# BogdanDIA/gr-dvbt

Hardware: AMD Instinct MI355X
Metric: RX Msamples/s (baseband in -> TS out) (higher is better)
Workload: dtype u8 (Viterbi/RS) + f32 (front end)

## Files before the change

gr_dvbt_amd/csrc/k_symbol8k.hpp:

```cpp
#pragma once
#include "k_frontend.hpp"
#include "k_backend.hpp"

namespace dvbt {

#ifndef S8_EXP
#define S8_EXP 0
#endif
#ifndef S8_MIN_WAVES
#define S8_MIN_WAVES 4
#endif
constexpr int S8_N = 8192, S8_T = 512, S8_PAY = 6048, S8_NCP = 177, S8_NTPS = 68, S8_ZL = 688;
constexpr int S8_IT = (S8_PAY + S8_T - 1) / S8_T;
#ifndef S8_TOP_N
#define S8_TOP_N 6
#endif
constexpr int S8_TOP = S8_TOP_N;
constexpr size_t S8_SMALL_BYTES = DEMOD_NP * 8 + 2 * 128 * 8 + 64 * 8 + 192 * 4 + 16 * 4 + 64 * 4 + 192 * 2 + 64 + 16;
constexpr size_t S8_LDS_BYTES = (size_t)((S8_EXP & 128) ? S8_N / 2 : S8_N) * 8 + S8_SMALL_BYTES;
#ifndef S8_WG_PER_CU
#define S8_WG_PER_CU 2
#endif
inline int s8_grid(int cus) { return S8_WG_PER_CU * cus; }

__device__ __forceinline__ int s8_swz1(int a) { return a ^ ((a >> 5) & 15) ^ (((a >> 9) & 1) << 4); }
__device__ __forceinline__ int s8_swz2(int b) { return b ^ ((b >> 4) & 15); }

__device__ __forceinline__ void s8_fill_ptab(float2 *pt, const SymMeta &m, int t)
{
  const double thA = (double)m.ph_base + m.incA, thB = (double)m.ph_base + (double)m.sw * (m.incA - m.incB) + m.incB;
  double ang;
  if (t < 16) ang = 512.0 * t * m.incA;
  else if (t < 32) ang = 512.0 * (t - 16) * m.incB;
  else if (t < 48) ang = thA + 32.0 * (t - 32) * m.incA;
  else if (t < 64) ang = thB + 32.0 * (t - 48) * m.incB;
  else if (t < 96) ang = (double)(t - 64) * m.incA;
  else ang = (double)(t - 96) * m.incB;
  float sn, cs; sincosf(wrap_pi(ang), &sn, &cs);
  pt[t] = make_float2(cs, sn);
}

typedef float v2f __attribute__((ext_vector_type(2)));
__device__ __forceinline__ v2f s8_v(float2 a) { return (v2f){a.x, a.y}; }
__device__ __forceinline__ float2 s8_f(v2f a) { return make_float2(a.x, a.y); }
__device__ __forceinline__ v2f s8_cmul(v2f a, v2f b)
{
  v2f p, r;
  asm("v_pk_mul_f32 %0, %1, %2 op_sel:[1,1] op_sel_hi:[1,0]" : "=v"(p) : "v"(a), "v"(b));
  asm("v_pk_fma_f32 %0, %1, %2, %3 op_sel:[0,0,0] op_sel_hi:[0,1,1] neg_lo:[0,0,1]" : "=v"(r) : "v"(a), "v"(b), "v"(p));
  return r;
}
__device__ __forceinline__ v2f s8_add_mi(v2f a, v2f b)
{ v2f r; asm("v_pk_add_f32 %0, %1, %2 op_sel:[0,1] op_sel_hi:[1,0] neg_hi:[0,1]" : "=v"(r) : "v"(a), "v"(b)); return r; }
__device__ __forceinline__ v2f s8_add_pi(v2f a, v2f b)
{ v2f r; asm("v_pk_add_f32 %0, %1, %2 op_sel:[0,1] op_sel_hi:[1,0] neg_lo:[0,1]" : "=v"(r) : "v"(a), "v"(b)); return r; }
__device__ __forceinline__ v2f s8_mul_mi(v2f y)
{ v2f r; asm("v_pk_add_f32 %0, %1, 0 op_sel:[1,0] op_sel_hi:[0,1] neg_hi:[1,0]" : "=v"(r) : "v"(y)); return r; }
#define S8_MULK(name, m1, m2) \
  __device__ __forceinline__ v2f name(v2f y, v2f K) { v2f p, r; \
    asm("v_pk_mul_f32 %0, %1, %2 " m1 : "=v"(p) : "v"(y), "v"(K)); \
    asm("v_pk_fma_f32 %0, %1, %2, %3 " m2 : "=v"(r) : "v"(y), "v"(K), "v"(p)); return r; }
S8_MULK(s8_mul_c_ms, "op_sel:[0,0] op_sel_hi:[1,0]", "op_sel:[1,1,0] op_sel_hi:[0,1,1] neg_hi:[1,0,0]")
S8_MULK(s8_mul_s_mc, "op_sel:[0,1] op_sel_hi:[1,1]", "op_sel:[1,0,0] op_sel_hi:[0,0,1] neg_hi:[1,0,0]")
S8_MULK(s8_mul_mc_s, "op_sel:[0,0] op_sel_hi:[1,0] neg_lo:[0,1] neg_hi:[0,1]", "op_sel:[1,1,0] op_sel_hi:[0,1,1] neg_lo:[1,0,0]")
S8_MULK(s8_mul_ms_mc, "op_sel:[0,1] op_sel_hi:[1,1] neg_lo:[0,1] neg_hi:[0,1]", "op_sel:[1,0,0] op_sel_hi:[0,0,1] neg_hi:[1,0,0]")
S8_MULK(s8_mul_mc_ms, "op_sel:[0,0] op_sel_hi:[1,0] neg_lo:[0,1] neg_hi:[0,1]", "op_sel:[1,1,0] op_sel_hi:[0,1,1] neg_hi:[1,0,0]")
#undef S8_MULK
__device__ __forceinline__ v2f s8_mul_h_mh(v2f y, v2f H)
{
  v2f t, r;
  asm("v_pk_add_f32 %0, %1, %1 op_sel:[0,1] op_sel_hi:[1,0] neg_hi:[0,1]" : "=v"(t) : "v"(y));
  asm("v_pk_mul_f32 %0, %1, %2" : "=v"(r) : "v"(t), "v"(H));
  return r;
}
__device__ __forceinline__ v2f s8_mul_mh_mh(v2f y, v2f H)
{
  v2f t, r;
  asm("v_pk_add_f32 %0, %1, %1 op_sel:[0,1] op_sel_hi:[1,0] neg_lo:[0,1]" : "=v"(t) : "v"(y));
  asm("v_pk_mul_f32 %0, %1, %2 neg_lo:[0,1] neg_hi:[0,1]" : "=v"(r) : "v"(t), "v"(H));
  return r;
}
struct S8Roots { v2f K8, K16, K316, H; };
__device__ __forceinline__ S8Roots s8_roots()
{
  S8Roots R;
  R.K8 = (v2f){0.92387953251128674f, 0.38268343236508977f}; R.K16 = (v2f){0.98078528040323043f, 0.19509032201612825f};
  R.K316 = (v2f){0.83146961230254524f, 0.55557023301960218f}; R.H = (v2f){0.70710678118654752f, 0.70710678118654752f};
  return R;
}
__device__ __forceinline__ void s8_bfly4(v2f a0, v2f a1, v2f a2, v2f a3, v2f &y0, v2f &y1, v2f &y2, v2f &y3)
{
  const v2f s02 = a0 + a2, d02 = a0 - a2, s13 = a1 + a3, d13 = a1 - a3;
  y0 = s02 + s13; y2 = s02 - s13; y1 = s8_add_mi(d02, d13); y3 = s8_add_pi(d02, d13);
}
__device__ __forceinline__ void s8_dft16(v2f (&a)[16], const S8Roots &R)
{
  v2f t[16];
#pragma unroll
  for (int rp = 0; rp < 4; rp++) {
    v2f y0, y1, y2, y3;
    s8_bfly4(a[rp], a[rp + 4], a[rp + 8], a[rp + 12], y0, y1, y2, y3);
    t[rp] = y0;
    if (rp == 0) { t[4] = y1; t[8] = y2; t[12] = y3; }
    else if (rp == 1) { t[5] = s8_mul_c_ms(y1, R.K8); t[9] = s8_mul_h_mh(y2, R.H); t[13] = s8_mul_s_mc(y3, R.K8); }
    else if (rp == 2) { t[6] = s8_mul_h_mh(y1, R.H); t[10] = s8_mul_mi(y2); t[14] = s8_mul_mh_mh(y3, R.H); }
    else { t[7] = s8_mul_s_mc(y1, R.K8); t[11] = s8_mul_mh_mh(y2, R.H); t[15] = s8_mul_mc_s(y3, R.K8); }
  }
#pragma unroll
  for (int k1 = 0; k1 < 4; k1++) {
    v2f y0, y1, y2, y3;
    s8_bfly4(t[k1 * 4], t[k1 * 4 + 1], t[k1 * 4 + 2], t[k1 * 4 + 3], y0, y1, y2, y3);
    a[k1] = y0; a[k1 + 4] = y1; a[k1 + 8] = y2; a[k1 + 12] = y3;
  }
}
__device__ __forceinline__ void s8_twiddle16(v2f (&a)[16], v2f w1)
{
  v2f w[16];
  w[1] = w1;
  w[2] = s8_cmul(w[1], w[1]); w[3] = s8_cmul(w[2], w[1]); w[4] = s8_cmul(w[2], w[2]); w[5] = s8_cmul(w[4], w[1]); w[6] = s8_cmul(w[3], w[3]);
  w[7] = s8_cmul(w[4], w[3]); w[8] = s8_cmul(w[4], w[4]); w[9] = s8_cmul(w[8], w[1]); w[10] = s8_cmul(w[5], w[5]); w[11] = s8_cmul(w[8], w[3]);
  w[12] = s8_cmul(w[6], w[6]); w[13] = s8_cmul(w[8], w[5]); w[14] = s8_cmul(w[7], w[7]); w[15] = s8_cmul(w[8], w[7]);
#pragma unroll
  for (int k = 1; k < 16; k++) a[k] = s8_cmul(a[k], w[k]);
}
template <int B> __device__ __forceinline__ v2f s8_mul_w32(v2f u, const S8Roots &R)
{
  if (B == 1) return s8_mul_c_ms(u, R.K16); if (B == 2) return s8_mul_c_ms(u, R.K8); if (B == 3) return s8_mul_c_ms(u, R.K316);
  if (B == 4) return s8_mul_h_mh(u, R.H);
  if (B == 5) return s8_mul_s_mc(u, R.K316); if (B == 6) return s8_mul_s_mc(u, R.K8); if (B == 7) return s8_mul_s_mc(u, R.K16);
  if (B == 8) return s8_mul_mi(u);
  if (B == 9) return s8_mul_ms_mc(u, R.K16); if (B == 10) return s8_mul_ms_mc(u, R.K8); if (B == 11) return s8_mul_ms_mc(u, R.K316);
  if (B == 12) return s8_mul_mh_mh(u, R.H);
  if (B == 13) return s8_mul_mc_ms(u, R.K316); if (B == 14) return s8_mul_mc_ms(u, R.K8); if (B == 15) return s8_mul_mc_ms(u, R.K16);
  return u;
}

template <int CTRL> __device__ __forceinline__ float s8_dpp(float v) { return __builtin_bit_cast(float, __builtin_amdgcn_update_dpp(0, __builtin_bit_cast(int, v), CTRL, 0xf, 0xf, true)); }
__device__ __forceinline__ float s8_row_sum(float v)
{ v += s8_dpp<0xB1>(v); v += s8_dpp<0x4E>(v); v += s8_dpp<0x141>(v); v += s8_dpp<0x140>(v); return v; }
__device__ __forceinline__ float s8_row_max(float v)
{ v = fmaxf(v, s8_dpp<0xB1>(v)); v = fmaxf(v, s8_dpp<0x4E>(v)); v = fmaxf(v, s8_dpp<0x141>(v)); v = fmaxf(v, s8_dpp<0x140>(v)); return v; }
__device__ __forceinline__ float s8_quad_max(float v) { v = fmaxf(v, s8_dpp<0xB1>(v)); return fmaxf(v, s8_dpp<0x4E>(v)); }

constexpr float S8_MARGIN = 2.0e-5f, S8_REACH = 4.0f;
__device__ __forceinline__ bool s8_demap_cell(v2f e, float inv_step, float half_n, float top, int &idx)
{
  const float gx = __builtin_fmaf(e.x, inv_step, half_n), gy = __builtin_fmaf(e.y, inv_step, half_n);
  const float cx = __builtin_amdgcn_fmed3f(gx, 0.5f, top), cy = __builtin_amdgcn_fmed3f(gy, 0.5f, top);
  const float fx = floorf(cx), fy = floorf(cy);
  const bool ok = fabsf((cx - fx) - 0.5f) < 0.5f - S8_MARGIN && fabsf((cy - fy) - 0.5f) < 0.5f - S8_MARGIN &&
                  fabsf(gx - cx) < S8_REACH && fabsf(gy - cy) < S8_REACH;
  idx = (int)fx * 8 + (int)fy;
  return ok;
}

typedef int s8_i4 __attribute__((ext_vector_type(4)));
__device__ v2f s8_raw_buffer_load_v2f32(s8_i4 rsrc, int voffset, int soffset, int aux) __asm("llvm.amdgcn.raw.buffer.load.v2f32");
__device__ __forceinline__ s8_i4 s8_rsrc(const v2f *base)
{
  const unsigned long long a = (unsigned long long)base;
  s8_i4 r;
  r.x = __builtin_amdgcn_readfirstlane((int)(unsigned)a); r.y = __builtin_amdgcn_readfirstlane((int)(unsigned)(a >> 32)) & 0xffff;
  r.z = 0x7fffffff; r.w = 0x00020000;
  return r;
}
__device__ __forceinline__ s8_i4 s8_rsrc_lim(const v2f *iq, long long low, long long avail)
{
  s8_i4 r = s8_rsrc(iq + low);
  long long bytes = (avail - low) * 8; bytes = bytes < 0 ? 0 : (bytes > 0x7fffffffll ? 0x7fffffffll : bytes);
  r.z = __builtin_amdgcn_readfirstlane((int)bytes);
  return r;
}
__device__ __forceinline__ v2f s8_sample(s8_i4 rsrc, int i, int tid) { return s8_raw_buffer_load_v2f32(rsrc, tid * 8, i * S8_T * 8, 0); }

template <bool TAPS, bool DRIFT> __global__ __launch_bounds__(S8_T, S8_MIN_WAVES) void symbol8k_kernel(const float2 *__restrict__ iq_, FrontParams p, const RxState *st,
                                                           const SymMeta *__restrict__ meta, const float2 *__restrict__ tw, float2 *__restrict__ acq_tap,
                                                           float2 *__restrict__ fft_tap, DemodTables T, float2 *__restrict__ eq_tap,
                                                           float2 *__restrict__ tpsval, SymInfo *__restrict__ info, InnerParams ip,
                                                           const float2 *__restrict__ points, const unsigned char *__restrict__ label_tab,
                                                           uint8_t *__restrict__ labels, int *__restrict__ ticket,
                                                           const float *__restrict__ drift, const int *__restrict__ drift_flags, float *__restrict__ csi_tap)
{
  if ((drift_flags[1] != 0) != DRIFT) return;
  extern __shared__ __attribute__((aligned(16))) unsigned char smem_raw[];
  v2f *x = reinterpret_cast<v2f *>((S8_EXP & 128) ? smem_raw + S8_SMALL_BYTES : smem_raw);
  v2f *gtab = (S8_EXP & 128) ? reinterpret_cast<v2f *>(smem_raw) : x + S8_N;
  float2 *ptab = reinterpret_cast<float2 *>(gtab + DEMOD_NP);
  float2 *pts = ptab + 256;
  float *s_known = reinterpret_cast<float *>(pts + 64);
  float *s_cfo = s_known + 192;
  float *s_pat = s_cfo + 16;
  short *s_cpil = reinterpret_cast<short *>(s_pat + 64);
  unsigned char *label_of = reinterpret_cast<unsigned char *>(s_cpil + 192);
  int *s_tkt = reinterpret_cast<int *>(label_of + 64);
  const v2f *iq = reinterpret_cast<const v2f *>(iq_);
  constexpr int N = S8_N, zl = S8_ZL;
  const int tid0 = threadIdx.x, tid = tid0, cp = p.cp;
  const int nsym = st->n_symbols, call0 = st->call0;
  if (tid == 0) s_tkt[0] = atomicAdd(ticket, 1);
  __syncthreads();
  int s = __builtin_amdgcn_readfirstlane(s_tkt[0]);
  if (s >= nsym) return;

  if (tid < 64) { pts[tid] = points[tid]; label_of[tid] = label_tab[tid]; }
  if (tid < S8_NCP) { s_cpil[tid] = T.cpilot[tid]; if (tid < S8_NCP - 1) s_known[tid] = T.known_diff[tid]; }
  const v2f w1A = s8_v(tw[tid]), w1B = s8_v(tw[16 * (tid & 31)]);
  const int tps_c = tid < S8_NTPS ? T.tps[tid] : 0;
  float pat_ref = 0.f;
  if (tid >= 256) { const int q = tid - 256, j = q & 15, pat = (q >> 4) & 3; if (j < 10) pat_ref = T.pilot_ref[3 * pat + 12 * j]; }
  const float half_n = 0.5f * (float)ip.nlev, top = (float)ip.nlev - 0.5f;

  int cur_mod = 0, s_prev = s;

  SymMeta m = meta[s];
  v2f vin[16];
  {
    const long long low = (long long)(call0 + s) * (N + cp) + m.cp_start - N + 1;
    const s8_i4 rs = s8_rsrc_lim(iq, low, p.avail);
#pragma unroll
    for (int i = S8_TOP; i < 16; i++) vin[i] = s8_sample(rs, i, tid);
  }
  if (tid < 128) s8_fill_ptab(ptab, m, tid);
  int par = 0;
  __syncthreads();

  for (;;) {
    int tid = tid0;
    asm volatile("" : "+v"(tid));
    const S8Roots R = s8_roots();
    int tkt = 0;
    if (tid == 0) tkt = atomicAdd(ticket, 1);
    const bool last = !p.keep_last && s + 1 >= nsym;
    {
      const long long low = (long long)(call0 + s) * (N + cp) + m.cp_start - N + 1;
      const s8_i4 rs = s8_rsrc_lim(iq, low, p.avail);
#pragma unroll
      for (int i = 0; i < ((S8_EXP & 4) ? 16 : S8_TOP); i++) vin[i] = s8_sample(rs, i, tid);
    }
    float dl[16];
    if (DRIFT) {
      const float *dt = drift + (size_t)s * (S8_N / 32) + (tid >> 5);
#pragma unroll
      for (int i = 0; i < 16; i++) dl[i] = dt[16 * i];
    }
    v2f a[16];
    {
      const v2f *pt = reinterpret_cast<const v2f *>(ptab) + par * 128;
      const v2f PA = s8_cmul(pt[32 + (tid >> 5)], pt[64 + (tid & 31)]), PB = s8_cmul(pt[48 + (tid >> 5)], pt[96 + (tid & 31)]);
      const int sw = (m.sw >= 0 && m.sw < N + cp) ? m.sw : 0x7fffffff;
#pragma unroll
      for (int k = 0; k < 16; k++) {
        const int i = (k + S8_TOP) & 15, n = tid + i * S8_T;
        const bool pieceB = n + 1 > sw;
        const v2f P = pieceB ? PB : PA;
        a[i] = (S8_EXP & 32) ? vin[i] : s8_cmul(s8_cmul(P, pt[(pieceB ? 16 : 0) + i]), vin[i]);
        if (DRIFT) a[i] = (v2f){__builtin_fmaf(-dl[i], a[i].y, a[i].x), __builtin_fmaf(dl[i], a[i].x, a[i].y)};
        if (TAPS && acq_tap) acq_tap[(size_t)s * N + n] = s8_f(a[i]);
      }
    }
    s8_dft16(a, R);
    { v2f wA = w1A; asm volatile("" : "+v"(wA), "+v"(a[15]));
      s8_twiddle16(a, wA); }
    __syncthreads();
    {
      const int b0 = tid ^ ((tid >> 5) & 15);
#pragma unroll
      for (int k1 = 0; k1 < 16; k1++) x[k1 * 512 + (b0 ^ ((k1 & 1) << 4))] = a[k1];
    }
    __syncthreads();
    if (!(S8_EXP & 2)) {
    {
      const int k1 = tid >> 5, mm = (tid & 31) ^ ((k1 & 1) << 4), rb = k1 * 512;
#pragma unroll
      for (int m1 = 0; m1 < 16; m1++) a[m1] = x[rb + 32 * m1 + (mm ^ m1)];
      s8_dft16(a, R);
      { v2f wB = w1B; asm volatile("" : "+v"(wB), "+v"(a[15]));
        s8_twiddle16(a, wB); }
#pragma unroll
      for (int j1 = 0; j1 < 16; j1++) x[rb + 32 * j1 + (mm ^ j1)] = a[j1];
    }
    __syncthreads();
    {
      const int j1 = tid & 15, k1 = (tid >> 4) & 15, c = tid >> 8, jj = j1 ^ ((k1 & 1) << 4), rb = k1 * 512 + 32 * j1;
      if (c == 0) {
#pragma unroll
        for (int b = 0; b < 16; b++) a[b] = x[rb + (b ^ jj)] + x[rb + ((b + 16) ^ jj)];
      } else {
        v2f u[16];
#pragma unroll
        for (int b = 0; b < 16; b++) u[b] = x[rb + (b ^ jj)] - x[rb + ((b + 16) ^ jj)];
        a[0] = u[0];
        a[1] = s8_mul_w32<1>(u[1], R); a[2] = s8_mul_w32<2>(u[2], R); a[3] = s8_mul_w32<3>(u[3], R); a[4] = s8_mul_w32<4>(u[4], R);
        a[5] = s8_mul_w32<5>(u[5], R); a[6] = s8_mul_w32<6>(u[6], R); a[7] = s8_mul_w32<7>(u[7], R); a[8] = s8_mul_w32<8>(u[8], R);
        a[9] = s8_mul_w32<9>(u[9], R); a[10] = s8_mul_w32<10>(u[10], R); a[11] = s8_mul_w32<11>(u[11], R); a[12] = s8_mul_w32<12>(u[12], R);
        a[13] = s8_mul_w32<13>(u[13], R); a[14] = s8_mul_w32<14>(u[14], R); a[15] = s8_mul_w32<15>(u[15], R);
      }
      s8_dft16(a, R);
      __syncthreads();
      const int base2 = (k1 ^ j1) + 16 * j1 + 256 * c;
#pragma unroll
      for (int d = 0; d < 16; d++) x[base2 + 512 * (d ^ 8)] = a[d];
    }
    }
    if (tid == 0) s_tkt[1] = tkt;
    __syncthreads();
    const int s_next = __builtin_amdgcn_readfirstlane(s_tkt[1]);
    const bool more = s_next < nsym;
    SymMeta mn = m;
    if (more) mn = meta[s_next];
    auto X = [&](int b) -> v2f { return x[s8_swz2(b)]; };
    unsigned tcl[S8_IT];
    unsigned est0 = 0, est1 = 0, tps_l = 0, tps_dd = 0; int np = 0;
    auto load_rows = [&](int md) {
      const uint32_t *pp = T.pay_pack + (size_t)md * S8_PAY;
#pragma unroll
      for (int it = 0; it < S8_IT; it++) { const int i = tid + it * S8_T; tcl[it] = pp[i < S8_PAY ? i : S8_PAY - 1]; }
      np = md == 0 ? T.np[0] : md == 1 ? T.np[1] : md == 2 ? T.np[2] : T.np[3];
      const uint16_t *pk = T.pil_k + (size_t)md * DEMOD_NP;
      est0 = pk[tid < np ? tid : 0]; est1 = pk[tid + S8_T < np ? tid + S8_T : 0];
      if (tid < S8_NTPS) { const int q = md * S8_NTPS + tid; tps_l = T.tps_Li[q]; tps_dd = T.tps_d[q]; }
    };
    const int pred = (cur_mod + (s - s_prev)) & 3;
    if (!last && !(S8_EXP & 1)) load_rows(pred);
    if (TAPS && fft_tap) {
#pragma unroll
      for (int i = 0; i < 16; i++) { const int b = tid + i * S8_T; fft_tap[(size_t)s * N + b] = s8_f(X(b)); }
    }
    if (last) break;
    if (S8_EXP & 1) {
      if (more) {
        const long long low = (long long)(call0 + s_next) * (N + cp) + mn.cp_start - N + 1;
        const s8_i4 rs = s8_rsrc_lim(iq, low, p.avail);
#pragma unroll
        for (int i = S8_TOP; i < 16; i++) vin[i] = s8_sample(rs, i, tid);
      }
      if (x[tid].x == 123.f) labels[s] = 1;
      if (!more) break;
      s = s_next; m = mn; par ^= 1;
      continue;
    }

    if (S8_EXP & 16) { if (tid < 80) s_cfo[tid] = tid == 8 ? 1.f : 0.f; }
    else if (tid < 256) {
      const int cand = tid >> 4, sub = tid & 15, i = zl - 8 + cand;
      constexpr int NJ = (S8_NCP - 1) / 16;
      int c0[NJ], c1[NJ]; v2f u[NJ], v[NJ];
#pragma unroll
      for (int k = 0; k < NJ; k++) { c0[k] = s_cpil[sub + 16 * k]; c1[k] = s_cpil[sub + 16 * k + 1]; }
#pragma unroll
      for (int k = 0; k < NJ; k++) { u[k] = X(i + c1[k]); v[k] = X(i + c0[k]); }
      float sum = 0.f;
#pragma unroll
      for (int k = 0; k < NJ; k++) { const v2f d = u[k] - v[k]; sum += s_known[sub + 16 * k] * (d.x * d.x + d.y * d.y); }
      sum = s8_row_sum(sum);
      if (sub == 0) s_cfo[cand] = sum;
    } else {
      const int q = tid - 256, j = q & 15, pat = (q >> 4) & 3, cg = q >> 6;
      v2f v[4];
#pragma unroll
      for (int cc = 0; cc < 4; cc++) v[cc] = X(zl - 8 + cg * 4 + cc + 3 * pat + 12 * (j < 10 ? j : 0));
#pragma unroll
      for (int cc = 0; cc < 4; cc++) {
        const float cr = s8_row_sum(j < 10 ? pat_ref * v[cc].x : 0.f), ci = s8_row_sum(j < 10 ? -pat_ref * v[cc].y : 0.f);
        if (j == 0) s_pat[(cg * 4 + cc) * 4 + pat] = cr * cr + ci * ci;
      }
      if (more && q < 128) s8_fill_ptab(ptab + (par ^ 1) * 128, mn, q);
    }
    __syncthreads();
    int fo, mod;
    {
      const int l = tid & 63;
      float v = s_cfo[l & 15];
      float mx = s8_row_max(v);
      const unsigned long long hit = __ballot(v == mx && mx > 0.f && l < 16);
      const int best = hit ? __builtin_ctzll(hit) : 8;
      v = s_pat[best * 4 + (l & 3)];
      mx = s8_quad_max(v);
      const unsigned long long hit2 = __ballot(v == mx && mx > 0.f && l < 4);
      fo = best - 8; mod = hit2 ? __builtin_ctzll(hit2) : 0;
    }
    const int xb = zl + fo;
    if (tid == 0) { SymInfo si; si.freq_offset = fo; si.mod_index = mod; si.cfc = 0.f; si.pad = 0; info[s] = si; }
    if (more && !(S8_EXP & (4 | 64))) {
      const long long low = (long long)(call0 + s_next) * (N + cp) + mn.cp_start - N + 1;
      const s8_i4 rs = s8_rsrc_lim(iq, low, p.avail);
#pragma unroll
      for (int i = S8_TOP; i < 16; i++) vin[i] = s8_sample(rs, i, tid);
    }
    if (mod != pred) load_rows(mod);
    cur_mod = mod; s_prev = s;
    {
      const float amp = (float)(4.0 / 3.0);
#pragma unroll
      for (int h = 0; h < 2; h++) {
        const int e = (int)(h ? est1 : est0), r = tid + h * S8_T;
        if (r < np) {
          const v2f v = X(xb + (e & 0x7fff));
          const float q = ((e & 0x8000) ? -amp : amp) * __builtin_amdgcn_rcpf(v.x * v.x + v.y * v.y);
          gtab[r] = (v2f){q * v.x, -q * v.y};
        }
      }
    }
    __syncthreads();
    auto equalise = [&](int c, int Li, int dj) -> v2f {
      const v2f gl = gtab[Li], gr = gtab[Li + 1];
      const float k11 = 1.0f / 11.0f, j = (float)dj;
      const v2f t = (gr - gl) * k11;
      return s8_cmul(X(xb + c), (v2f){__builtin_fmaf(t.x, j, gl.x), __builtin_fmaf(t.y, j, gl.y)});
    };
    {
      uint8_t *lab = labels + (size_t)s * S8_PAY;
      bool slow = ip.hshift != 0.f;
#pragma unroll
      for (int it = 0; it < S8_IT; it++) {
        const int i = tid + it * S8_T;
        if ((it < S8_PAY / S8_T || i < S8_PAY) && !(S8_EXP & 8)) {
          const v2f e = equalise((int)(tcl[it] & 0x1fffu), (int)((tcl[it] >> 13) & 0x3ffu), (int)(tcl[it] >> 23));
          if (TAPS && eq_tap) eq_tap[(size_t)s * S8_PAY + i] = s8_f(e);
          if (TAPS && csi_tap) {
            const int Li = (int)((tcl[it] >> 13) & 0x3ffu); const float j = (float)(tcl[it] >> 23);
            const v2f gl = gtab[Li], gr = gtab[Li + 1], t2 = (gr - gl) * (1.0f / 11.0f);
            const float gx = __builtin_fmaf(t2.x, j, gl.x), gy = __builtin_fmaf(t2.y, j, gl.y);
            csi_tap[(size_t)s * S8_PAY + i] = 1.0f / (gx * gx + gy * gy);
          }
          int idx;
          const bool cell_ok = s8_demap_cell(e, ip.inv_step, half_n, top, idx);
          if (!(S8_EXP & 128)) slow |= !cell_ok;
          lab[i] = label_of[idx & 63];
        }
#ifdef S8_BATCH
        if (it % S8_BATCH == S8_BATCH - 1) __builtin_amdgcn_sched_barrier(0);
#endif
      }
      if (__any(slow)) {
#pragma unroll 1
        for (int it = 0; it < S8_IT; it++) {
          const int i = tid + it * S8_T;
          if (i >= S8_PAY) break;
          const unsigned w = T.pay_pack[(size_t)mod * S8_PAY + i];
          const v2f e = equalise((int)(w & 0x1fffu), (int)((w >> 13) & 0x3ffu), (int)(w >> 23));
          int f = demap_fast(s8_f(e), pts, label_of, ip);
          if (f < 0) f = demap_all(s8_f(e), pts, ip.csize);
          lab[i] = (uint8_t)f;
        }
      }
    }
    if (more && (S8_EXP & 64)) {
      const long long low = (long long)(call0 + s_next) * (N + cp) + mn.cp_start - N + 1;
      const s8_i4 rs = s8_rsrc_lim(iq, low, p.avail);
#pragma unroll
      for (int i = S8_TOP; i < 16; i++) vin[i] = s8_sample(rs, i, tid);
    }
    if (tid < S8_NTPS)
      tpsval[(size_t)s * S8_NTPS + tid] = s8_f(equalise(tps_c, (int)tps_l, (int)tps_dd));
    if (!more) break;
    s = s_next; m = mn; par ^= 1;
  }
}

}
```

Before: 40720.

## Specialize CP phase pieces per wave, precompute CFO LDS addresses, buffer-load payload rows

Adds S8_PARTS-gated micro-optimizations to the 8k symbol kernel. When the whole wave sits on one side of the phase switch point, it applies a single phase piece and skips the per-sample select. It precomputes swizzled LDS byte addresses for the CFO candidate correlation into a shared table and computes FFT-pass LDS addresses with xor on a base address. Payload-row loads switch to bounds-checked raw buffer loads. These cut VALU address arithmetic and selects, but the address table takes more LDS and the per-wave branches may add divergence overhead.

```diff
diff --git a/gr_dvbt_amd/csrc/k_symbol8k.hpp b/gr_dvbt_amd/csrc/k_symbol8k.hpp
--- a/gr_dvbt_amd/csrc/k_symbol8k.hpp
+++ b/gr_dvbt_amd/csrc/k_symbol8k.hpp
@@ -16,8 +16,15 @@
 #define S8_TOP_N 6
 #endif
 constexpr int S8_TOP = S8_TOP_N;
-constexpr size_t S8_SMALL_BYTES = DEMOD_NP * 8 + 2 * 128 * 8 + 64 * 8 + 192 * 4 + 16 * 4 + 64 * 4 + 192 * 2 + 64 + 16;
+#ifndef S8_PARTS
+#define S8_PARTS ((S8_EXP & 128) ? 7 : 15)
+#endif
+constexpr int S8_NCAND = 16;
+constexpr size_t S8_CFOA_BYTES = (S8_PARTS & 2) ? S8_NCAND * S8_NCP * 2 : 192 * 2;
+constexpr size_t S8_SMALL_BYTES = DEMOD_NP * 8 + 2 * 128 * 8 + 64 * 8 + 192 * 4 + 16 * 4 + 64 * 4 + S8_CFOA_BYTES + 64 + 16;
 constexpr size_t S8_LDS_BYTES = (size_t)((S8_EXP & 128) ? S8_N / 2 : S8_N) * 8 + S8_SMALL_BYTES;
+static_assert(S8_LDS_BYTES <= 81920, "two workgroups per CU: 160 KB of LDS");
+static_assert(S8_CFOA_BYTES % 16 == 0, "label_of and s_tkt behind the table stay aligned");
 #ifndef S8_WG_PER_CU
 #define S8_WG_PER_CU 2
 #endif
@@ -25,6 +32,7 @@
 
 __device__ __forceinline__ int s8_swz1(int a) { return a ^ ((a >> 5) & 15) ^ (((a >> 9) & 1) << 4); }
 __device__ __forceinline__ int s8_swz2(int b) { return b ^ ((b >> 4) & 15); }
+__device__ __forceinline__ unsigned short s8_cfo_addr(int cand, int carrier, unsigned image) { return (unsigned short)(image + s8_swz2(688 - 8 + cand + carrier) * 8); }
 
 __device__ __forceinline__ void s8_fill_ptab(float2 *pt, const SymMeta &m, int t)
 {
@@ -43,6 +51,9 @@
 typedef float v2f __attribute__((ext_vector_type(2)));
 __device__ __forceinline__ v2f s8_v(float2 a) { return (v2f){a.x, a.y}; }
 __device__ __forceinline__ float2 s8_f(v2f a) { return make_float2(a.x, a.y); }
+__device__ __forceinline__ unsigned s8_lds_addr(const void *q) { return (unsigned)(unsigned long long)(__attribute__((address_space(3))) const void *)q; }
+__device__ __forceinline__ v2f s8_lds_v2f(unsigned a) { return *(__attribute__((address_space(3))) const v2f *)(unsigned long long)a; }
+__device__ __forceinline__ void s8_lds_store(unsigned a, v2f v) { *(__attribute__((address_space(3))) v2f *)(unsigned long long)a = v; }
 __device__ __forceinline__ v2f s8_cmul(v2f a, v2f b)
 {
   v2f p, r;
@@ -172,6 +183,8 @@
   return r;
 }
 __device__ __forceinline__ v2f s8_sample(s8_i4 rsrc, int i, int tid) { return s8_raw_buffer_load_v2f32(rsrc, tid * 8, i * S8_T * 8, 0); }
+__device__ unsigned s8_raw_buffer_load_u32(s8_i4 rsrc, int voffset, int soffset, int aux) __asm("llvm.amdgcn.raw.buffer.load.i32");
+__device__ __forceinline__ s8_i4 s8_rsrc_rows(const uint32_t *rows) { s8_i4 r = s8_rsrc(reinterpret_cast<const v2f *>(rows)); r.z = S8_PAY * 4; return r; }
 
 template <bool TAPS, bool DRIFT> __global__ __launch_bounds__(S8_T, S8_MIN_WAVES) void symbol8k_kernel(const float2 *__restrict__ iq_, FrontParams p, const RxState *st,
                                                            const SymMeta *__restrict__ meta, const float2 *__restrict__ tw, float2 *__restrict__ acq_tap,
@@ -182,7 +195,7 @@
                                                            const float *__restrict__ drift, const int *__restrict__ drift_flags, float *__restrict__ csi_tap)
 {
   if ((drift_flags[1] != 0) != DRIFT) return;
-  extern __shared__ __attribute__((aligned(16))) unsigned char smem_raw[];
+  extern __shared__ __attribute__((aligned(128))) unsigned char smem_raw[];
   v2f *x = reinterpret_cast<v2f *>((S8_EXP & 128) ? smem_raw + S8_SMALL_BYTES : smem_raw);
   v2f *gtab = (S8_EXP & 128) ? reinterpret_cast<v2f *>(smem_raw) : x + S8_N;
   float2 *ptab = reinterpret_cast<float2 *>(gtab + DEMOD_NP);
@@ -191,7 +204,8 @@
   float *s_cfo = s_known + 192;
   float *s_pat = s_cfo + 16;
   short *s_cpil = reinterpret_cast<short *>(s_pat + 64);
-  unsigned char *label_of = reinterpret_cast<unsigned char *>(s_cpil + 192);
+  unsigned short *s_cfoa = reinterpret_cast<unsigned short *>(s_pat + 64);
+  unsigned char *label_of = reinterpret_cast<unsigned char *>(s_pat + 64) + S8_CFOA_BYTES;
   int *s_tkt = reinterpret_cast<int *>(label_of + 64);
   const v2f *iq = reinterpret_cast<const v2f *>(iq_);
   constexpr int N = S8_N, zl = S8_ZL;
@@ -203,7 +217,10 @@
   if (s >= nsym) return;
 
   if (tid < 64) { pts[tid] = points[tid]; label_of[tid] = label_tab[tid]; }
-  if (tid < S8_NCP) { s_cpil[tid] = T.cpilot[tid]; if (tid < S8_NCP - 1) s_known[tid] = T.known_diff[tid]; }
+  if (tid < S8_NCP - 1) s_known[tid] = T.known_diff[tid];
+  if (S8_PARTS & 2) { for (int e = tid; e < S8_NCAND * S8_NCP; e += S8_T) s_cfoa[e] = s8_cfo_addr(e / S8_NCP, T.cpilot[e % S8_NCP], s8_lds_addr(x)); }
+  else if (tid < S8_NCP) s_cpil[tid] = T.cpilot[tid];
+  const int wave0 = __builtin_amdgcn_readfirstlane(tid0) & ~63;
   const v2f w1A = s8_v(tw[tid]), w1B = s8_v(tw[16 * (tid & 31)]);
   const int tps_c = tid < S8_NTPS ? T.tps[tid] : 0;
   float pat_ref = 0.f;
@@ -228,6 +245,8 @@
     int tid = tid0;
     asm volatile("" : "+v"(tid));
     const S8Roots R = s8_roots();
+    int t_hi = tid >> 5, t_lo = tid & 31;
+    asm volatile("" : "+v"(t_hi), "+v"(t_lo));
     int tkt = 0;
     if (tid == 0) tkt = atomicAdd(ticket, 1);
     const bool last = !p.keep_last && s + 1 >= nsym;
@@ -246,14 +265,25 @@
     v2f a[16];
     {
       const v2f *pt = reinterpret_cast<const v2f *>(ptab) + par * 128;
-      const v2f PA = s8_cmul(pt[32 + (tid >> 5)], pt[64 + (tid & 31)]), PB = s8_cmul(pt[48 + (tid >> 5)], pt[96 + (tid & 31)]);
+      const v2f PA = s8_cmul(pt[32 + t_hi], pt[64 + t_lo]), PB = s8_cmul(pt[48 + t_hi], pt[96 + t_lo]);
       const int sw = (m.sw >= 0 && m.sw < N + cp) ? m.sw : 0x7fffffff;
+      const int swd = sw - wave0;
 #pragma unroll
       for (int k = 0; k < 16; k++) {
         const int i = (k + S8_TOP) & 15, n = tid + i * S8_T;
-        const bool pieceB = n + 1 > sw;
-        const v2f P = pieceB ? PB : PA;
-        a[i] = (S8_EXP & 32) ? vin[i] : s8_cmul(s8_cmul(P, pt[(pieceB ? 16 : 0) + i]), vin[i]);
+        if (S8_EXP & 32) a[i] = vin[i];
+        else if ((S8_PARTS & 1) && swd >= i * S8_T + 64) { a[i] = s8_cmul(s8_cmul(PA, pt[i]), vin[i]); asm volatile("; piece A" : "+v"(a[i])); }
+        else if ((S8_PARTS & 1) && swd <= i * S8_T) { a[i] = s8_cmul(s8_cmul(PB, pt[16 + i]), vin[i]); asm volatile("; piece B" : "+v"(a[i])); }
+        else {
+          const bool pieceB = n + 1 > sw;
+          const v2f P = pieceB ? PB : PA;
+          a[i] = s8_cmul(s8_cmul(P, pt[(pieceB ? 16 : 0) + i]), vin[i]);
+          asm volatile("; both pieces" : "+v"(a[i]));
+        }
+      }
+#pragma unroll
+      for (int k = 0; k < 16; k++) {
+        const int i = (k + S8_TOP) & 15, n = tid + i * S8_T;
         if (DRIFT) a[i] = (v2f){__builtin_fmaf(-dl[i], a[i].y, a[i].x), __builtin_fmaf(dl[i], a[i].x, a[i].y)};
         if (TAPS && acq_tap) acq_tap[(size_t)s * N + n] = s8_f(a[i]);
       }
@@ -263,21 +293,22 @@
       s8_twiddle16(a, wA); }
     __syncthreads();
     {
-      const int b0 = tid ^ ((tid >> 5) & 15);
+      const int b0 = tid ^ (t_hi & 15);
 #pragma unroll
       for (int k1 = 0; k1 < 16; k1++) x[k1 * 512 + (b0 ^ ((k1 & 1) << 4))] = a[k1];
     }
     __syncthreads();
     if (!(S8_EXP & 2)) {
     {
-      const int k1 = tid >> 5, mm = (tid & 31) ^ ((k1 & 1) << 4), rb = k1 * 512;
-#pragma unroll
-      for (int m1 = 0; m1 < 16; m1++) a[m1] = x[rb + 32 * m1 + (mm ^ m1)];
+      const int k1 = t_hi, mm = t_lo ^ ((k1 & 1) << 4), rb = k1 * 512;
+      const unsigned tb = s8_lds_addr(x) + (unsigned)(rb + mm) * 8;
+#pragma unroll
+      for (int m1 = 0; m1 < 16; m1++) a[m1] = (S8_PARTS & 8) ? s8_lds_v2f((tb ^ (m1 * 8)) + 256 * m1) : x[rb + 32 * m1 + (mm ^ m1)];
       s8_dft16(a, R);
       { v2f wB = w1B; asm volatile("" : "+v"(wB), "+v"(a[15]));
         s8_twiddle16(a, wB); }
 #pragma unroll
-      for (int j1 = 0; j1 < 16; j1++) x[rb + 32 * j1 + (mm ^ j1)] = a[j1];
+      for (int j1 = 0; j1 < 16; j1++) { if (S8_PARTS & 8) s8_lds_store((tb ^ (j1 * 8)) + 256 * j1, a[j1]); else x[rb + 32 * j1 + (mm ^ j1)] = a[j1]; }
     }
     __syncthreads();
     {
@@ -313,8 +344,14 @@
     unsigned est0 = 0, est1 = 0, tps_l = 0, tps_dd = 0; int np = 0;
     auto load_rows = [&](int md) {
       const uint32_t *pp = T.pay_pack + (size_t)md * S8_PAY;
-#pragma unroll
-      for (int it = 0; it < S8_IT; it++) { const int i = tid + it * S8_T; tcl[it] = pp[i < S8_PAY ? i : S8_PAY - 1]; }
+      if (S8_PARTS & 4) {
+        const s8_i4 rr = s8_rsrc_rows(pp);
+#pragma unroll
+        for (int it = 0; it < S8_IT; it++) tcl[it] = s8_raw_buffer_load_u32(rr, tid * 4, it * S8_T * 4, 0);
+      } else {
+#pragma unroll
+        for (int it = 0; it < S8_IT; it++) { const int i = tid + it * S8_T; tcl[it] = pp[i < S8_PAY ? i : S8_PAY - 1]; }
+      }
       np = md == 0 ? T.np[0] : md == 1 ? T.np[1] : md == 2 ? T.np[2] : T.np[3];
       const uint16_t *pk = T.pil_k + (size_t)md * DEMOD_NP;
       est0 = pk[tid < np ? tid : 0]; est1 = pk[tid + S8_T < np ? tid + S8_T : 0];
@@ -345,10 +382,18 @@
       const int cand = tid >> 4, sub = tid & 15, i = zl - 8 + cand;
       constexpr int NJ = (S8_NCP - 1) / 16;
       int c0[NJ], c1[NJ]; v2f u[NJ], v[NJ];
-#pragma unroll
-      for (int k = 0; k < NJ; k++) { c0[k] = s_cpil[sub + 16 * k]; c1[k] = s_cpil[sub + 16 * k + 1]; }
-#pragma unroll
-      for (int k = 0; k < NJ; k++) { u[k] = X(i + c1[k]); v[k] = X(i + c0[k]); }
+      if (S8_PARTS & 2) {
+        const unsigned short *ca = s_cfoa + cand * S8_NCP + sub;
+#pragma unroll
+        for (int k = 0; k < NJ; k++) { c0[k] = ca[16 * k]; c1[k] = ca[16 * k + 1]; }
+#pragma unroll
+        for (int k = 0; k < NJ; k++) { u[k] = s8_lds_v2f(c1[k]); v[k] = s8_lds_v2f(c0[k]); }
+      } else {
+#pragma unroll
+        for (int k = 0; k < NJ; k++) { c0[k] = s_cpil[sub + 16 * k]; c1[k] = s_cpil[sub + 16 * k + 1]; }
+#pragma unroll
+        for (int k = 0; k < NJ; k++) { u[k] = X(i + c1[k]); v[k] = X(i + c0[k]); }
+      }
       float sum = 0.f;
 #pragma unroll
       for (int k = 0; k < NJ; k++) { const v2f d = u[k] - v[k]; sum += s_known[sub + 16 * k] * (d.x * d.x + d.y * d.y); }
```

New measurement: 40940 (median of 6 runs). No clear change (+0.5%).
